# argumentcomputer/multi-stark

Measured on AMD Instinct MI355X. Metric: prove_trace_rows_per_sec, higher is better.
Workload: dtype u64; 1 GPU; U32-add + byte-table lookup (benches/multi_stark.rs), 2^20 additions per proof, bench_config(): log_blowup 2, 100 queries, 10+10 PoW bits, GoldilocksBlake3Config; witness (traces + claims, 64-bit words) in pinned host memory at step start: upload, from_stage_1 on the device and read-back inside the timed region; the library narrows byte-valued traces on host threads INSIDE the step before they cro; rows_per_proof=1048832, proof_bytes=1100053, parallelism=single GPU

## Files before the change

### multi-stark_amd/csrc/host.h

```cpp
#pragma once
#include <memory>
#include <vector>

#include "../../include/mstark.h"
#include "b3_dev.h"
#include "msamd.h"
#include "program.h"

namespace msamd {

void blake3_host(const uint8_t* in, size_t len, uint8_t out[32]);
std::string last_error_text();

struct Challenger {
  std::vector<uint8_t> input, output;
  explicit Challenger(const std::vector<uint8_t>& seed) : input(seed) {}
  void observe_bytes(const uint8_t* p, size_t n) {
    output.clear();
    input.insert(input.end(), p, p + n);
  }
  void observe(u64 v) {
    uint8_t b[8];
    for (int k = 0; k < 8; k++) b[k] = (uint8_t)(v >> (8 * k));
    observe_bytes(b, 8);
// ... 39 lines not shown
  DProgram prog;
  DProgram prefix_prog;
  JitKernel stage2_jit;
  JitKernel stage2_trace_jit;
  bool prefix_on_device = false;
  size_t quotient_degree() const {
    size_t d = (max_constraint_degree > 2 ? max_constraint_degree : 2) - 1, q = 1;
    while (q < d) q <<= 1;
    return q;
  }
};

struct PcsData {
  std::vector<DMat> ldes;
  DTree tree;
};

struct HSystem {
  Ctx* ctx = nullptr;
  Params params;
  std::vector<HCircuit> circuits;
  bool has_pre = false;
  std::vector<Digest> pre_commit;
  std::vector<int> pre_indices;
  PcsData pre_data;
  std::vector<uint8_t> seed;
};
std::unique_ptr<HSystem> system_from_blob(Ctx& ctx, const uint8_t* blob, size_t len);

struct HWitness {
  HSystem* sys = nullptr;
  std::vector<size_t> heights;
  std::vector<DBuf<u64>> traces;
  bool has_remote = false;
  std::vector<DLookups> lookups;
  std::vector<u64> claim_offsets, claim_data;
  size_t claim_elem0 = 0, claim_elems_total = 0;
  std::vector<u64> claim_head;
  bool claims_partial = false;
  DBuf<u64> d_claim_offsets, d_claim_data;
  bool host_resident = false;
  std::vector<const u64*> h_traces;
  std::vector<std::vector<u64>> h_mult, h_args;
  std::vector<void*> registered;
  std::vector<unsigned> pack_bytes;
  std::vector<uint8_t*> h_packed;
  struct Staged {
    bool valid = false, has_host_lookups = false;
    std::vector<DBuf<u64>> traces, mult, args;
    DBuf<u64> claim_offsets, claim_data;
    hipEvent_t ev[3] = {nullptr, nullptr, nullptr};
    void clear() {
      valid = false;
      traces.clear();
      mult.clear();
      args.clear();
      claim_offsets.reset();
      claim_data.reset();
    }
  };
  Staged stage[2];
  int cur = 0;
  bool prefetch = false;
  bool pinned = true;
  void pin(const void* p, size_t bytes);
  HWitness() {}
  HWitness(const HWitness&) = delete;
  HWitness& operator=(const HWitness&) = delete;
  ~HWitness();
};
std::unique_ptr<HWitness> witness_create_host(HSystem& sys, const u64* const* traces, const u64* heights, size_t n_claims,
                                              const u64* claim_offsets, const u64* claim_data, size_t data_first = 0,
                                              size_t data_count = ~size_t(0), const u64* head = nullptr, size_t n_head = 0);
void claims_slice_range(const HSystem& sys, const size_t* heights, size_t n_claims, const u64* offsets, size_t rank, size_t world, size_t& first,
                        size_t& count);
std::unique_ptr<HWitness> witness_create(HSystem& sys, const u64* const* traces, const u64* heights, const u64* const* mult,
                                         const u64* const* args, size_t n_claims, const u64* claim_offsets,
                                         const u64* claim_data);

struct ReadyLookups {
  DBuf<u64> mult, args;
};
std::unique_ptr<HWitness> witness_from_device(HSystem& sys, std::vector<DBuf<u64>>&& traces, const std::vector<size_t>& heights,
                                              DBuf<u64>&& d_claim_offsets, DBuf<u64>&& d_claim_data, size_t n_claims, size_t claim_elems,
                                              std::vector<ReadyLookups>* ready = nullptr);
std::unique_ptr<HWitness> witness_create_device(HSystem& sys, const ms_dev_matrix* traces, size_t n_claims, const u64* claim_offsets,
                                                const u64* claim_data, bool claims_on_device, void* producer_stream);
// ... 50 lines not shown
```

### multi-stark_amd/csrc/msamd.h

```cpp
#pragma once
#include <hip/hip_runtime.h>

#include <algorithm>
#include <cstdint>
#include <cstring>
#include <map>
#include <mutex>
#include <stdexcept>
#include <string>
#include <vector>

#include "gl_dev.h"

namespace msamd {

#define HIP_CHECK(expr)                                                                                   \
  do {                                                                                                    \
    hipError_t _e = (expr);                                                                               \
    if (_e != hipSuccess)                                                                                 \
      throw std::runtime_error(std::string("HIP error: ") + hipGetErrorString(_e) + " at " + __FILE__ + ":" + \
                               std::to_string(__LINE__));                                                 \
  } while (0)

static constexpr unsigned TW_LOG = 28;
// ... 160 lines not shown
  DBuf& operator=(DBuf&& o) noexcept {
    if (this != &o) {
      reset();
      ctx = o.ctx;
      p = o.p;
      n = o.n;
      o.p = nullptr;
    }
    return *this;
  }
  void reset() {
    if (p && ctx) ctx->release(p);
    p = nullptr;
  }
  ~DBuf() { reset(); }
};

struct DMat {
  DBuf<u64> buf;
  size_t h = 0, w = 0;
  u64* d() const { return buf.p; }
};

struct NttSrc {
  const u64* src = nullptr;
  unsigned src_div = 1;
  const u64* scale = nullptr;
};
void ntt_dif(Ctx& ctx, u64* data, unsigned logn, size_t ncols, bool inverse, const NttSrc* from = nullptr, u64 out_mul = 1);
void ntt_dit(Ctx& ctx, u64* data, unsigned logn, size_t ncols, bool inverse, u64 out_mul = 1);
void transpose_in(Ctx& ctx, const u64* rowmajor, u64* colmajor, size_t h, size_t w, bool bitrev_rows);
void transpose_out(Ctx& ctx, const u64* colmajor, u64* rowmajor, size_t h, size_t w, bool bitrev_rows);
void pull_widen_words(const uint8_t* host_packed, unsigned bytes, size_t count, u64* out, hipStream_t stream);
void lde_from_coeffs(Ctx& ctx, const u64* coef, u64* lde, unsigned logn, unsigned log_blowup, size_t w);
void coset_lde(Ctx& ctx, u64* evals_bitrev, u64* lde, unsigned logn, unsigned log_blowup, size_t w);
void quotient_lde(Ctx& ctx, u64* qvals_bitrev, u64* lde, unsigned logn, unsigned logq, unsigned log_blowup, size_t D);

struct MatRef {
  const u64* d;
  uint32_t w;
  uint32_t pad;
  uint64_t stride;
};
struct DTree {
  std::vector<const u64*> mat_d;
  std::vector<size_t> mat_h, mat_w;
  std::vector<size_t> mat_stride;
  DBuf<Digest> digests;
  Digest* ext = nullptr;
  Digest* base() const { return ext ? ext : digests.p; }
  std::vector<size_t> layer_off, layer_len;
  unsigned cap_height = 0;
  size_t max_height() const { return layer_len.empty() ? 0 : layer_len[0]; }
  size_t cap_layer() const {
    size_t L = layer_len.size();
    size_t ch = cap_height < L - 1 ? cap_height : L - 1;
    return L - 1 - ch;
  }
};
void merkle_build(Ctx& ctx, DTree& t);
void merkle_alloc(Ctx& ctx, DTree& t, size_t max_height);
struct FriChallenge;
void merkle_compress_plain(Ctx& ctx, DTree& t, const FriChallenge* fc = nullptr);
std::vector<Digest> merkle_cap(Ctx& ctx, const DTree& t);
void merkle_tree_top(Ctx& ctx, const Digest* d_roots, size_t n, Digest* d_out);
Digest blake3_device(Ctx& ctx, const uint8_t* d_prefix, size_t prefix_len, const u64* d_words, size_t nwords);
// ... 210 lines not shown
```

### multi-stark_amd/csrc/ntt.hip

```cpp
#include <cstring>

#include "msamd.h"

namespace msamd {

namespace {

__device__ __forceinline__ u64 tw_lookup(const u64* __restrict__ t0, const u64* __restrict__ t1, u32 e26) {
  return gl_mul(t1[e26 >> TW_HALF], t0[e26 & ((1u << TW_HALF) - 1)]);
}

template <int DIT>
__device__ __forceinline__ void lds_stages(u64* sm, unsigned k, unsigned logT, const u64* __restrict__ t1) {
  if (k == 0) return;
  const unsigned T = 1u << logT;
  const unsigned nb = (1u << (k - 1)) << logT;
  for (unsigned s = 0; s < k; s++) {
    const unsigned loghalf = DIT ? s : (k - 1 - s);
    const unsigned half = 1u << loghalf;
    const unsigned tsh = TW_HALF - loghalf - 1;
    for (unsigned b = threadIdx.x; b < nb; b += blockDim.x) {
      unsigned l = b & (T - 1), bb = b >> logT;
      unsigned j = bb & (half - 1), grp = bb >> loghalf;
      unsigned i0 = (((grp << (loghalf + 1)) + j) << logT) + l;
// ... 798 lines not shown
    if (sizeof(T) == 1) {
#pragma unroll
      for (int k = 0; k < 4; k++) {
        o[2 * k] = make_ulonglong2(w[k] & 0xff, (w[k] >> 8) & 0xff);
        o[2 * k + 1] = make_ulonglong2((w[k] >> 16) & 0xff, w[k] >> 24);
      }
    } else if (sizeof(T) == 2) {
#pragma unroll
      for (int k = 0; k < 4; k++) o[k] = make_ulonglong2(w[k] & 0xffff, w[k] >> 16);
    } else {
      o[0] = make_ulonglong2(w[0], w[1]);
      o[1] = make_ulonglong2(w[2], w[3]);
    }
  }
  if (blockIdx.x == 0 && threadIdx.x == 0)
    for (size_t k = whole; k < count; k++) out[k] = host[k];
}
}
void pull_widen_words(const uint8_t* host_packed, unsigned bytes, size_t count, u64* out, hipStream_t stream) {
  if (!count) return;
  if (reinterpret_cast<uintptr_t>(host_packed) & 15) throw std::runtime_error("pull_widen_words: source must be 16-byte aligned");
  const dim3 grid((unsigned)std::min<size_t>(256, (count * bytes / 16 + 255) / 256 + 1)), block(256);
  if (bytes == 1)
    hipLaunchKernelGGL(pull_widen_k<uint8_t>, grid, block, 0, stream, host_packed, count, out);
  else if (bytes == 2)
    hipLaunchKernelGGL(pull_widen_k<uint16_t>, grid, block, 0, stream, reinterpret_cast<const uint16_t*>(host_packed), count, out);
  else if (bytes == 4)
    hipLaunchKernelGGL(pull_widen_k<uint32_t>, grid, block, 0, stream, reinterpret_cast<const uint32_t*>(host_packed), count, out);
  else
    throw std::runtime_error("pull_widen_words: unsupported width");
  HIP_CHECK(hipGetLastError());
}

void transpose_out(Ctx& ctx, const u64* colmajor, u64* rowmajor, size_t h, size_t w, bool bitrev_rows) {
  if (h * w == 0) return;
  hipLaunchKernelGGL(transpose_out_k, dim3((unsigned)((h * w + 255) / 256)), dim3(256), 0, ctx.stream, colmajor, rowmajor, h,
                     w, log2_strict(h), bitrev_rows ? 1 : 0);
  HIP_CHECK(hipGetLastError());
}

}
```

### multi-stark_amd/csrc/prover.hip

```cpp
#include <algorithm>
#include <chrono>
#include <cstdio>
#include <cstdlib>

#include <sys/resource.h>
#include <unistd.h>

#include <atomic>
#include <condition_variable>
#include <functional>
#include <mutex>
#include <thread>

#include "host.h"
#include "ingest.h"
#include "lookup_params.h"
#include "open_plan.h"
#include "quotient_params.h"

namespace msamd {

namespace {
void load_block(const uint8_t* p, size_t len, u32 w[16]) {
  uint8_t buf[64];
// ... 127 lines not shown
  size_t n, off = 0;
  u64 word() {
    if (off + 8 > n) throw std::runtime_error("system blob truncated");
    u64 v;
    memcpy(&v, p + off, 8);
    off += 8;
    return v;
  }
};
const u64 BLOB_MAGIC = 0x31305359534D0000ULL;
}

void commit_matrices(Ctx& ctx, std::vector<DMat>&& ldes, unsigned cap_height, PcsData& out) {
  out.ldes = std::move(ldes);
  out.tree = DTree();
  out.tree.cap_height = cap_height;
  for (auto& m : out.ldes) {
    out.tree.mat_d.push_back(m.d());
    out.tree.mat_h.push_back(m.h);
    out.tree.mat_w.push_back(m.w);
  }
  merkle_build(ctx, out.tree);
}

static DMat lde_of_host_matrix(Ctx& ctx, const u64* rowmajor_dev, size_t h, size_t w, unsigned lb) {
  unsigned logn = log2_strict(h);
  DBuf<u64> ev(ctx, h * w);
  transpose_in(ctx, rowmajor_dev, ev.p, h, w, true);
  DMat lde;
  lde.h = h << lb;
  lde.w = w;
  lde.buf = DBuf<u64>(ctx, lde.h * w);
  coset_lde(ctx, ev.p, lde.d(), logn, lb, w);
  return lde;
}

std::unique_ptr<HSystem> system_from_blob(Ctx& ctx, const uint8_t* blob, size_t len) {
  HIP_CHECK(hipSetDevice(ctx.device));
  Reader rd{blob, len};
  if (rd.word() != BLOB_MAGIC) throw std::runtime_error("bad system blob magic");
  std::unique_ptr<HSystem> sys(new HSystem());
  sys->ctx = &ctx;
  Params& p = sys->params;
  p.log_blowup = rd.word();
  p.cap_height = rd.word();
  p.log_final_poly_len = rd.word();
  p.max_log_arity = rd.word();
  p.num_queries = rd.word();
  p.commit_pow_bits = rd.word();
  p.query_pow_bits = rd.word();
  if (p.max_log_arity < 1 || p.max_log_arity > FRI_MAX_LOG_ARITY) throw std::runtime_error("max_log_arity must be 1 .. 6 (a FRI row is hashed as one BLAKE3 chunk)");
  if (p.log_blowup < 1 || p.log_blowup > 8) throw std::runtime_error("log_blowup out of range");
  if (p.commit_pow_bits > 40 || p.query_pow_bits > 40) throw std::runtime_error("proof-of-work bits out of range");
  {
    const char* tag = "multi-stark/v0";
    sys->seed.assign(tag, tag + 14);
    const u64 ps[7] = {p.log_blowup, p.cap_height, p.log_final_poly_len, p.max_log_arity, p.num_queries, p.commit_pow_bits,
                       p.query_pow_bits};
    for (u64 x : ps)
      for (int k = 0; k < 8; k++) sys->seed.push_back((uint8_t)(x >> (8 * k)));
  }
  const size_t D = 2;
  size_t nc = rd.word();
  std::vector<DMat> pre_ldes;
  for (size_t ci = 0; ci < nc; ci++) {
    sys->circuits.emplace_back();
// ... 373 lines not shown
  w->claim_elems_total = tot;
  for (u64 x : w->claim_data)
    if (x >= GL_P) throw std::runtime_error("non-canonical claim value");
  w->d_claim_offsets = DBuf<u64>(ctx, n_claims + 1);
  w->d_claim_data = DBuf<u64>(ctx, std::max<size_t>(tot, 1));
  ctx.h2d(w->d_claim_offsets.p, w->claim_offsets.data(), (n_claims + 1) * 8);
  if (tot) ctx.h2d(w->d_claim_data.p, w->claim_data.data(), tot * 8);
  ctx.sync();
  return w;
}

u64 narrow_range(const u64* in, uint8_t* out, unsigned pb, size_t n);
namespace {
class PackPool {
 public:
  static PackPool* get(int device) {
    static std::mutex mu;
    static std::map<int, PackPool*> pools;
    static const int n_threads = []() {
      int n = 16;
      if (const char* e = getenv("MSAMD_PACK_THREADS")) n = atoi(e);
      return n > 64 ? 64 : n;
    }();
    if (n_threads <= 0) return nullptr;
    std::lock_guard<std::mutex> lk(mu);
    auto it = pools.find(device);
    if (it != pools.end()) return it->second;
    PackPool* p = new PackPool(n_threads);
    pools[device] = p;
    return p;
  }
  static constexpr size_t MAX_CHUNKS = 64, MAX_SUB = 128;
  size_t n_chunks = 0;
  void start(const u64* in, uint8_t* out, unsigned pb, size_t cnt, size_t chunks) {
    job_mu_.lock();
    std::unique_lock<std::mutex> lk(mu_);
    done_cv_.wait(lk, [&] { return busy_ == 0; });
    in_ = in, out_ = out, pb_ = pb, cnt_ = cnt;
    caller_ = std::this_thread::get_id();
    straggle_us_ = getenv("MSAMD_PACK_STRAGGLE_US") ? (unsigned)atoi(getenv("MSAMD_PACK_STRAGGLE_US")) : 0;
    n_chunks = std::max<size_t>(1, std::min(chunks, MAX_CHUNKS));
    per_chunk_ = ((cnt + n_chunks - 1) / n_chunks + 63) & ~size_t(63);
    n_chunks = (cnt + per_chunk_ - 1) / per_chunk_;
    next_.store(0);
    acc_.store(0);
    nsub_ = std::min<size_t>(2 * threads_.size(), MAX_SUB);
    for (size_t k = 0; k < n_chunks; k++) left_[k].store((int)nsub_);
    for (size_t i = 0; i < n_chunks * nsub_; i++) state_[i].store(0, std::memory_order_relaxed);
    busy_ = (int)threads_.size();
    gen_++;
    cv_.notify_all();
  }
  size_t chunk_begin(size_t k) const { return std::min(cnt_, k * per_chunk_); }
  bool wait_chunk(size_t k) {
    double all_claimed_at = 0;
    while (left_[k].load(std::memory_order_acquire) != 0) {
      if (next_.load(std::memory_order_relaxed) >= (k + 1) * nsub_) {
        const double now = now_ms();
        if (all_claimed_at == 0) all_claimed_at = now;
        if (now - all_claimed_at > 0.03) {
          for (size_t sub = 0; sub < nsub_ && left_[k].load(std::memory_order_acquire) != 0; sub++)
            if (state_[k * nsub_ + sub].load(std::memory_order_acquire) != 2) work_piece(k * nsub_ + sub, true);
          continue;
        }
      }
      if (!take_piece()) std::this_thread::yield();
    }
    return (acc_.load() >> (8 * pb_)) == 0;
  }
  void finish() { job_mu_.unlock(); }
  void quiesce() {
    std::unique_lock<std::mutex> lk(mu_);
    done_cv_.wait(lk, [&] { return busy_ == 0; });
  }
  struct Job {
    PackPool& p;
    Job(PackPool& pool, const u64* in, uint8_t* out, unsigned pb, size_t cnt, size_t chunks) : p(pool) { p.start(in, out, pb, cnt, chunks); }
    ~Job() { p.finish(); }
  };

 private:
  explicit PackPool(int n) {
    for (int i = 0; i < n; i++) threads_.emplace_back([this]() { run(); });
    for (auto& t : threads_) t.detach();
  }
  bool take_piece() {
    const size_t it = next_.fetch_add(1);
    if (it >= n_chunks * nsub_) return false;
    work_piece(it, false);
    return true;
  }
  void work_piece(size_t it, bool again) {
    const size_t k = it / nsub_, sub = it % nsub_;
    if (!again) {
      uint8_t unclaimed = 0;
      if (!state_[it].compare_exchange_strong(unclaimed, 1, std::memory_order_acq_rel)) return;
      if (straggle_us_ && sub == 3 && std::this_thread::get_id() != caller_)
        std::this_thread::sleep_for(std::chrono::microseconds(straggle_us_));
    }
    u64 acc = 0;
    const size_t b = chunk_begin(k), e = chunk_begin(k + 1);
    const size_t piece = (((e - b) + nsub_ - 1) / nsub_ + 7) & ~size_t(7);
    const size_t lo = std::min(e, b + sub * piece), hi = std::min(e, lo + piece);
    if (hi > lo) acc = narrow_range(in_ + lo, out_ + lo * pb_, pb_, hi - lo);
    if (acc) acc_.fetch_or(acc);
    if (state_[it].exchange(2, std::memory_order_acq_rel) != 2) left_[k].fetch_sub(1, std::memory_order_release);
  }
  void run() {
    uint64_t seen = 0;
    for (;;) {
      {
        std::unique_lock<std::mutex> lk(mu_);
        cv_.wait(lk, [&] { return gen_ != seen; });
        seen = gen_;
      }
      while (take_piece()) {
      }
      {
        std::unique_lock<std::mutex> lk(mu_);
        if (--busy_ == 0) done_cv_.notify_all();
      }
    }
  }
  std::vector<std::thread> threads_;
  std::mutex mu_, job_mu_;
  std::condition_variable cv_, done_cv_;
  uint64_t gen_ = 0;
  int busy_ = 0;
  const u64* in_ = nullptr;
  uint8_t* out_ = nullptr;
  unsigned pb_ = 1;
  size_t cnt_ = 0, per_chunk_ = 0, nsub_ = 1;
  std::atomic<uint8_t> state_[MAX_CHUNKS * MAX_SUB];
  std::thread::id caller_;
  unsigned straggle_us_ = 0;
  std::atomic<size_t> next_{0};
  std::atomic<u64> acc_{0};
  std::atomic<int> left_[MAX_CHUNKS];
};
}

void HWitness::pin(const void* p, size_t bytes) {
  if (!p || !bytes) return;
  const int r = host_range_pin(p, bytes);
  if (r == 1)
    registered.push_back(const_cast<void*>(p));
  else if (r == 0)
    pinned = false;
}
HWitness::~HWitness() {
  if (!host_resident) return;
  if (sys && sys->ctx) {
    (void)hipSetDevice(sys->ctx->device);
    (void)hipStreamSynchronize(sys->ctx->copy_stream);
    (void)hipStreamSynchronize(sys->ctx->claims_stream);
    if (sys->ctx->side_stream) (void)hipStreamSynchronize(sys->ctx->side_stream);
    (void)hipStreamSynchronize(sys->ctx->main_stream);
  }
  for (auto& st : stage)
    for (auto& e : st.ev)
      if (e) (void)hipEventDestroy(e);
  bool any_packed = false;
  for (uint8_t* p : h_packed) any_packed = any_packed || p != nullptr;
  if (any_packed)
    if (PackPool* pool = PackPool::get(sys && sys->ctx ? sys->ctx->device : 0)) pool->quiesce();
// ... 74 lines not shown
  for (size_t i = 0; i < n_claims; i++)
    if (claim_offsets[i + 1] < claim_offsets[i]) throw std::runtime_error("claim offsets must be non-decreasing");
  const size_t tot = n_claims ? (size_t)claim_offsets[n_claims] : 0;
  w->claim_offsets.assign(claim_offsets, claim_offsets + n_claims + 1);
  w->claim_elems_total = tot;
  if (data_count == ~size_t(0)) {
    w->claim_data.assign(claim_data, claim_data + tot);
  } else {
    if (data_first > tot || data_count > tot - data_first) throw std::runtime_error("claims slice outside the claims' data");
    const size_t need_head = std::min<size_t>(tot, 130);
    if (n_head < need_head || (need_head && !head)) throw std::runtime_error("claims slice: the first 130 elements are needed on every rank");
    w->claims_partial = true;
    w->has_remote = true;
    w->claim_elem0 = data_first;
    w->claim_data.assign(claim_data, claim_data + data_count);
    w->claim_head.assign(head, head + need_head);
    for (u64 x : w->claim_head)
      if (x >= GL_P) throw std::runtime_error("non-canonical claim value");
  }
  for (u64 x : w->claim_data)
    if (x >= GL_P) throw std::runtime_error("non-canonical claim value");
  w->pin(w->claim_offsets.data(), (n_claims + 1) * 8);
  w->pin(w->claim_data.data(), w->claim_data.size() * 8);
  ctx.sync();
  return w;
}

namespace {
struct HostUpload {
  HWitness& w;
  Ctx& ctx;
  bool on = false;
  bool skip_claims = false;
  HostUpload(HWitness& wit, Ctx& c) : w(wit), ctx(c) {}
  bool fused(size_t ci) const {
    const HCircuit& c = w.sys->circuits[ci];
    return w.host_resident && c.stage2_trace_jit.function && w.h_mult[ci].empty();
  }
  void issue(HWitness::Staged& st) {
    HSystem& sys = *w.sys;
    const size_t C = sys.circuits.size();
    for (auto& e : st.ev)
      if (!e) HIP_CHECK(hipEventCreateWithFlags(&e, hipEventDisableTiming));
    st.clear();
    st.traces.resize(C);
    st.mult.resize(C);
    st.args.resize(C);
    HIP_CHECK(hipEventRecord(ctx.copy_ev[3], ctx.stream));
    HIP_CHECK(hipStreamWaitEvent(ctx.copy_stream, ctx.copy_ev[3], 0));
    ctx.side_config();
    ctx.copy_delay();
    HIP_CHECK(hipStreamWaitEvent(ctx.claims_stream, ctx.copy_ev[3], 0));
    const size_t n_claims = w.claim_offsets.size() - 1, tot = w.claim_data.size();
    auto from_caller = [&](void* dst, const void* src, size_t bytes, hipStream_t s) {
      if (w.pinned)
        HIP_CHECK(hipMemcpyAsync(dst, src, bytes, hipMemcpyHostToDevice, s));
      else
        ctx.bounce_h2d(dst, src, bytes, s);
    };
    for (size_t ci = 0; ci < C; ci++) {
      const HCircuit& c = sys.circuits[ci];
      const size_t h = w.heights[ci];
      if (!h || !w.h_traces[ci]) continue;
      const size_t cnt = h * c.main_width;
      st.traces[ci] = DBuf<u64>(ctx, cnt);
      const unsigned pb = w.pack_bytes[ci];
      PackPool* pool = pb && !w.prefetch ? PackPool::get(ctx.device) : nullptr;
      bool sent = false;
      if (pool) {
        static const size_t n_chunks = getenv("MSAMD_PACK_CHUNKS") ? (size_t)atoi(getenv("MSAMD_PACK_CHUNKS")) : 8;
        PackPool::Job job(*pool, w.h_traces[ci], w.h_packed[ci], pb, cnt, n_chunks);
        sent = true;
        for (size_t k = 0; k < pool->n_chunks; k++) {
          if (!pool->wait_chunk(k)) {
            sent = false;
            break;
          }
          if (k == 0) g_probes.mark("narrow upload: first chunk ready");
          const size_t b = pool->chunk_begin(k), e = pool->chunk_begin(k + 1);
          pull_widen_words(w.h_packed[ci] + b * pb, pb, e - b, st.traces[ci].p + b, ctx.copy_stream);
        }
        g_probes.mark("narrow upload: last chunk queued");
      }
      if (!sent) from_caller(st.traces[ci].p, w.h_traces[ci], cnt * 8, ctx.copy_stream);
    }
    HIP_CHECK(hipEventRecord(st.ev[0], ctx.copy_stream));
    st.has_host_lookups = false;
    for (size_t ci = 0; ci < C; ci++) {
      const HCircuit& c = sys.circuits[ci];
      const size_t h = w.heights[ci];
      if (!h || !c.num_lookups || !w.h_traces[ci]) continue;
      if (fused(ci)) continue;
      st.mult[ci] = DBuf<u64>(ctx, h * c.num_lookups);
      st.args[ci] = DBuf<u64>(ctx, std::max<size_t>(h * c.args_width, 1));
      if (!w.h_mult[ci].empty()) {
        st.has_host_lookups = true;
        from_caller(st.mult[ci].p, w.h_mult[ci].data(), w.h_mult[ci].size() * 8, ctx.copy_stream);
        if (!w.h_args[ci].empty()) from_caller(st.args[ci].p, w.h_args[ci].data(), w.h_args[ci].size() * 8, ctx.copy_stream);
      }
    }
    if (!skip_claims) {
      st.claim_offsets = DBuf<u64>(ctx, n_claims + 1);
      st.claim_data = DBuf<u64>(ctx, std::max<size_t>(tot, 1));
      from_caller(st.claim_offsets.p, w.claim_offsets.data(), (n_claims + 1) * 8, ctx.copy_stream);
      if (tot) from_caller(st.claim_data.p, w.claim_data.data(), tot * 8, ctx.copy_stream);
    }
    HIP_CHECK(hipEventRecord(st.ev[2], ctx.copy_stream));
    for (size_t ci = 0; ci < C; ci++) {
      const HCircuit& c = sys.circuits[ci];
      const size_t h = w.heights[ci];
      if (!h || !c.num_lookups || !w.h_mult[ci].empty() || fused(ci) || !w.h_traces[ci]) continue;
      if (!lookup_values_device(ctx, c.prefix_prog, st.traces[ci].p, c.pre_width ? c.d_preprocessed.p : nullptr, h, c.main_width, c.pre_width,
                                c.args_width, st.mult[ci].p, st.args[ci].p, ctx.copy_stream))
        throw std::runtime_error("host-resident witness: lookup prefix does not fit the device sweep");
    }
    HIP_CHECK(hipEventRecord(st.ev[1], ctx.copy_stream));
    st.valid = true;
  }
  void start() {
    if (!w.host_resident) return;
    on = true;
    if (w.prefetch && w.stage[w.cur ^ 1].valid)
      w.cur ^= 1;
    else
      issue(w.stage[w.cur]);
    HWitness::Staged& st = w.stage[w.cur];
    for (size_t ci = 0; ci < st.traces.size(); ci++) {
      w.traces[ci] = std::move(st.traces[ci]);
      w.lookups[ci].mult = std::move(st.mult[ci]);
      w.lookups[ci].args = std::move(st.args[ci]);
    }
    w.d_claim_offsets = std::move(st.claim_offsets);
    w.d_claim_data = std::move(st.claim_data);
    st.valid = false;
    if (w.prefetch) issue(w.stage[w.cur ^ 1]);
  }
  void wait_traces() {
    if (on) HIP_CHECK(hipStreamWaitEvent(ctx.stream, w.stage[w.cur].ev[0], 0));
  }
  void lookup_values() {
    if (!on) return;
    HIP_CHECK(hipStreamWaitEvent(ctx.stream, w.stage[w.cur].ev[1], 0));
    if (ctx.side_forked && ctx.stream != ctx.side_stream) HIP_CHECK(hipStreamWaitEvent(ctx.side_stream, w.stage[w.cur].ev[1], 0));
  }
  void wait_claims() {
    if (on) HIP_CHECK(hipStreamWaitEvent(ctx.stream, w.stage[w.cur].ev[2], 0));
  }
  ~HostUpload() {
    if (!on) return;
    (void)hipStreamSynchronize(ctx.copy_stream);
    (void)hipStreamSynchronize(ctx.claims_stream);
    for (auto& t : w.traces) t.reset();
    for (auto& lk : w.lookups) {
      lk.mult.reset();
      lk.args.reset();
    }
    w.d_claim_offsets.reset();
    w.d_claim_data.reset();
  }
};
}

namespace {
struct PW {
  std::vector<uint8_t> b;
  void u8(uint8_t x) { b.push_back(x); }
  void u64_(u64 x) {
    size_t o = b.size();
    b.resize(o + 8);
    memcpy(&b[o], &x, 8);
  }
  void ext(E2 e) {
    u64_(e.c0);
    u64_(e.c1);
  }
  void raw(const void* p, size_t n) {
    const uint8_t* q = (const uint8_t*)p;
    b.insert(b.end(), q, q + n);
  }
  void cap(const std::vector<Digest>& c) {
    u64_(c.size());
    for (auto& d : c) raw(d.b, 32);
  }
};
typedef std::vector<std::vector<std::vector<E2>>> OpenedRound;
// ... 868 lines not shown
  if (device_claims) {
    s1_cap.assign(ncap, Digest());
    if (sys.has_pre) ch.observe_cap(sys.pre_commit);
    cap_off = ch.input.size();
    ch.observe_cap(s1_cap);
    for (unsigned ld : log_degrees) ch.observe(ld);
    nchunks = blake3_num_chunks(ch.input.size(), claim_words);
    prefix_chunks = std::min(nchunks, (ch.input.size() + 1023) / 1024);
  }
  const bool late_chunk0 = device_claims && prefix_chunks == 1 && nchunks >= 2 && !getenv("MSAMD_OLD_CLAIMS_TREE");
  LateChunk0 late0;
  DBuf<uint8_t> d_prefix;
  auto claims_chunks = [&]() {
    up.wait_claims();
    d_words = DBuf<u64>(ctx, claim_words);
    claims_transcript_words(ctx, wit.d_claim_data.p, wit.d_claim_offsets.p, n_claims, claim_elems, d_words.p);
    d_cvs = DBuf<Digest>(ctx, nchunks);
    blake3_chunk_cvs(ctx, nullptr, ch.input.size(), d_words.p, claim_words, prefix_chunks, nchunks, d_cvs.p);
    d_prefix = DBuf<uint8_t>(ctx, ch.input.size());
    ctx.h2d(d_prefix.p, ch.input.data(), ch.input.size());
    if (late_chunk0) blake3_late_chunk0_prepare(ctx, d_cvs.p, nchunks, late0);
  };

  t0 = now_ms();
  RoctxRange phase("stark/stage1_commit");
  PcsData s1;
  {
    std::vector<DMat> ldes(NA);
    up.wait_traces();
    fork_side();
    for (size_t pos : order) {
      const size_t ci = aidx[pos];
      SideScope sc(ctx, on_side[pos]);
      ldes[pos] = lde_of_host_matrix(ctx, wit.traces[ci].p, wit.heights[ci], sys.circuits[ci].main_width, lb);
    }
    ctx.side_join();
    if (early_claims) {
      ctx.side_fork();
      SideScope sc(ctx, true);
      claims_chunks();
    }
    commit_matrices(ctx, std::move(ldes), (unsigned)prm.cap_height, s1);
  }
  g_probes.mark("stage 1 queued");
  up.wait_claims();
  if (!device_claims) {
    s1_cap = merkle_cap(ctx, s1.tree);
    lap(0);
    if (sys.has_pre) ch.observe_cap(sys.pre_commit);
    ch.observe_cap(s1_cap);
    for (unsigned ld : log_degrees) ch.observe(ld);
    ch.observe((u64)n_claims);
    for (size_t i = 0; i < n_claims; i++) {
      size_t a = wit.claim_offsets[i], b = wit.claim_offsets[i + 1];
      ch.observe((u64)(b - a));
      for (size_t k = a; k < b; k++) ch.observe(wit.claim_data[k]);
    }
  } else {
    lap(0);
    const size_t cl = s1.tree.cap_layer();
    if (s1.tree.layer_len[cl] != ncap) throw std::runtime_error("stage-1 cap size differs from the transcript's placeholder");
    const Digest* d_cap = s1.tree.base() + s1.tree.layer_off[cl];
    if (!early_claims) claims_chunks();
    ctx.side_join();
    od.digest = DBuf<Digest>(ctx, 1);
    if (dev_outer) {
      od.state = DBuf<u32>(ctx, 28);
      d_bg = DBuf<ChallengeBG>(ctx, 1);
    }
// ... 290 lines not shown
```

### multi-stark_amd/csrc/prover_sharded.inc

```

namespace {

struct Comm {
  Ctx& ctx;
  const ms_comm_t* c;
  bool ordered = false;
  const char* phase = "start";
  Comm(Ctx& x, const ms_comm_t* t) : ctx(x), c(t) {
    if (c->set_stream_ordered && !getenv("MSAMD_SHARDED_HOST_SYNC")) {
      if (c->set_stream_ordered(c->user, ctx.main_stream) != 0) throw std::runtime_error("ms_comm.set_stream_ordered failed");
      ordered = true;
    }
  }
  ~Comm() {
    if (ordered) (void)c->set_stream_ordered(c->user, nullptr);
  }
  Comm(const Comm&) = delete;
  Comm& operator=(const Comm&) = delete;
  struct Call {
    Ctx& ctx;
    Call(Comm& cm, const char* what, size_t bytes, size_t detail = 0) : ctx(cm.ctx) {
      char buf[200];
      snprintf(buf, sizeof(buf), "%s: %s (%zu bytes%s%s) on rank %d of %d", cm.phase, what, bytes, detail ? ", part " : "",
               detail ? std::to_string(detail).c_str() : "", cm.rank(), cm.world());
// ... 335 lines not shown
  const size_t total = n_claims ? (size_t)offsets[n_claims] : 0;
  const size_t claim_words = 1 + n_claims + total;
  if (claim_words <= 8192 || world <= 1) {
    first = 0;
    count = total;
    return;
  }
  size_t sl_lo, sl_hi, inv_lo, inv_hi;
  claims_cut(claims_prefix_len(sys, heights), claim_words, n_claims, offsets, world, rank, sl_lo, sl_hi, inv_lo, inv_hi);
  first = (size_t)offsets[sl_lo];
  count = (size_t)offsets[sl_hi] - first;
}

std::vector<uint8_t> prove_sharded(HSystem& sys, HWitness& wit, const ms_comm_t* comm, const int32_t* owners, StageMs* times) {
  Ctx& ctx = *sys.ctx;
  HIP_CHECK(hipSetDevice(ctx.device));
  Comm cm(ctx, comm);
  const Params& prm = sys.params;
  const unsigned lb = (unsigned)prm.log_blowup;
  const size_t C = sys.circuits.size();
  const size_t N = (size_t)cm.world(), me = (size_t)cm.rank();
  const unsigned lw = log2_world(cm.world());
  if (wit.sys != &sys || wit.heights.size() != C) throw std::runtime_error("witness does not belong to this system");
  double t_begin = now_ms(), t0;
  auto lap = [&](int slot) {
    if (times) {
      ctx.sync();
      times->v[slot] = now_ms() - t0;
    }
  };
  PhaseTrace tr(ctx);
  HostUpload up(wit, ctx);
  up.skip_claims = true;
  up.start();
  const size_t n_claims = wit.claim_offsets.size() - 1;
  const size_t claim_elems = wit.claim_elems_total;
  const size_t claim_words = 1 + n_claims + claim_elems;
  DBuf<u64> sl_offs, sl_data;
  size_t sl_lo = 0, sl_hi = 0, inv_lo = 0, inv_hi = 0;
  const bool sliced = wit.host_resident && claim_words > 8192;
  size_t n_active = 0;
  for (size_t i = 0; i < C; i++) n_active += wit.heights[i] > 0;
  size_t max_lde_log = 0;
  for (size_t i = 0; i < C; i++)
    if (wit.heights[i] > 0) max_lde_log = std::max<size_t>(max_lde_log, log2_strict(wit.heights[i]) + lb);
  const size_t cap_digests = size_t(1) << std::min<size_t>((size_t)prm.cap_height, max_lde_log);
  const size_t pl_expected = sys.seed.size() + 8 * (1 + 7 * C) + (sys.has_pre ? 32 * sys.pre_commit.size() : 0) + 32 * cap_digests + 8 * n_active;
  const bool dev_outer = claim_words > 8192 && outer_fits(cap_digests, n_active) && pl_expected <= 1024 &&
                         blake3_num_chunks(pl_expected, claim_words) >= 2 && !getenv("MSAMD_HOST_TRANSCRIPT");
  OuterDev od;
  LateChunk0 late0;
  if (sliced) {
    claims_cut(pl_expected, claim_words, n_claims, wit.claim_offsets.data(), N, me, sl_lo, sl_hi, inv_lo, inv_hi);
    const size_t cnt = sl_hi - sl_lo, o0 = (size_t)wit.claim_offsets[sl_lo], o1 = (size_t)wit.claim_offsets[sl_hi];
    sl_offs = DBuf<u64>(ctx, cnt + 1);
    sl_data = DBuf<u64>(ctx, std::max<size_t>(o1 - o0, 1));
    HIP_CHECK(hipEventRecord(ctx.copy_ev[3], ctx.stream));
    HIP_CHECK(hipStreamWaitEvent(ctx.copy_stream, ctx.copy_ev[3], 0));
    ctx.copy_delay();
    auto from_caller = [&](void* dst, const void* src, size_t bytes) {
      if (wit.pinned)
        HIP_CHECK(hipMemcpyAsync(dst, src, bytes, hipMemcpyHostToDevice, ctx.copy_stream));
      else
        ctx.bounce_h2d(dst, src, bytes, ctx.copy_stream);
    };
    from_caller(sl_offs.p, wit.claim_offsets.data() + sl_lo, (cnt + 1) * 8);
// ... 928 lines not shown
```

Baseline: 161.8 million rows/s.

## Fuse narrow-trace widening with bit-reversed column-major transpose during upload

Adds a kernel that pulls byte-packed trace tiles from pinned host memory and, in one pass, writes both the row-major trace and a bit-reversed column-major copy for the LDE. The host pack pool is changed to narrow rows in a tiled order that matches this kernel, and stage 1 builds the LDE straight from the prepared evaluations, skipping the separate transpose inside lde_of_host_matrix. This overlaps the transpose with the host-to-device transfer, at the cost of an extra full-size device buffer per trace and a more complex, strided access pattern on the host side. The sharded prover keeps the old path.

```diff
diff --git a/multi-stark_amd/csrc/host.h b/multi-stark_amd/csrc/host.h
--- a/multi-stark_amd/csrc/host.h
+++ b/multi-stark_amd/csrc/host.h
@@ -95,6 +95,8 @@
   HSystem* sys = nullptr;
   std::vector<size_t> heights;
   std::vector<DBuf<u64>> traces;
+  std::vector<DBuf<u64>> evals;
+  std::vector<char> evals_ok;
   bool has_remote = false;
   std::vector<DLookups> lookups;
   std::vector<u64> claim_offsets, claim_data;
@@ -111,11 +113,15 @@
   struct Staged {
     bool valid = false, has_host_lookups = false;
     std::vector<DBuf<u64>> traces, mult, args;
+    std::vector<DBuf<u64>> evals;
+    std::vector<char> evals_ok;
     DBuf<u64> claim_offsets, claim_data;
     hipEvent_t ev[3] = {nullptr, nullptr, nullptr};
     void clear() {
       valid = false;
       traces.clear();
+      evals.clear();
+      evals_ok.clear();
       mult.clear();
       args.clear();
       claim_offsets.reset();
diff --git a/multi-stark_amd/csrc/msamd.h b/multi-stark_amd/csrc/msamd.h
--- a/multi-stark_amd/csrc/msamd.h
+++ b/multi-stark_amd/csrc/msamd.h
@@ -216,6 +216,9 @@
 void transpose_in(Ctx& ctx, const u64* rowmajor, u64* colmajor, size_t h, size_t w, bool bitrev_rows);
 void transpose_out(Ctx& ctx, const u64* colmajor, u64* rowmajor, size_t h, size_t w, bool bitrev_rows);
 void pull_widen_words(const uint8_t* host_packed, unsigned bytes, size_t count, u64* out, hipStream_t stream);
+bool pull_widen_transpose_fits(size_t h, size_t w, unsigned bytes);
+void pull_widen_transpose(const uint8_t* host_packed, unsigned bytes, size_t h, size_t w, size_t m_begin, size_t m_end, u64* rowmajor,
+                          u64* colmajor, hipStream_t stream);
 void lde_from_coeffs(Ctx& ctx, const u64* coef, u64* lde, unsigned logn, unsigned log_blowup, size_t w);
 void coset_lde(Ctx& ctx, u64* evals_bitrev, u64* lde, unsigned logn, unsigned log_blowup, size_t w);
 void quotient_lde(Ctx& ctx, u64* qvals_bitrev, u64* lde, unsigned logn, unsigned logq, unsigned log_blowup, size_t D);
diff --git a/multi-stark_amd/csrc/ntt.hip b/multi-stark_amd/csrc/ntt.hip
--- a/multi-stark_amd/csrc/ntt.hip
+++ b/multi-stark_amd/csrc/ntt.hip
@@ -854,6 +854,86 @@
   HIP_CHECK(hipGetLastError());
 }
 
+namespace {
+template <class T>
+__global__ __launch_bounds__(256) void pull_widen_transpose_k(const uint4* __restrict__ host, u64* __restrict__ rowmajor,
+                                                              u64* __restrict__ colmajor, size_t h, u32 w, unsigned logh, u32 m_begin,
+                                                              u32 m_end) {
+  constexpr u32 PER = 16 / sizeof(T), SLAB = 16;
+  __shared__ uint4 stage[16 * SLAB];
+  typedef T __attribute__((may_alias)) TA;
+  const TA* tile = reinterpret_cast<const TA*>(stage);
+  const u32 t = threadIdx.x;
+  const u32 q = w * (u32)sizeof(T);
+  const size_t len = size_t(m_end - m_begin) * q;
+  const size_t items = (len + SLAB - 1) / SLAB;
+  const u32 d16 = 16 / w, s16 = 16 - d16 * w;
+  auto load = [&](size_t item) {
+    const size_t s0 = item * SLAB;
+    const u32 cnt = (u32)min(size_t(SLAB), len - s0);
+    const u32 u = t / cnt, j = t - u * cnt;
+    return t < 16 * cnt ? host[((size_t(u) << (logh - 8)) + m_begin) * q + s0 + j] : make_uint4(0, 0, 0, 0);
+  };
+  size_t item = blockIdx.x;
+  uint4 v = make_uint4(0, 0, 0, 0);
+  if (item < items) v = load(item);
+  for (; item < items; item += gridDim.x) {
+    const size_t s0 = item * SLAB;
+    const u32 cnt = (u32)min(size_t(SLAB), len - s0);
+    if (t < 16 * cnt) stage[t] = v;
+    __syncthreads();
+    if (item + gridDim.x < items) v = load(item + gridDim.x);
+    const u32 ne = cnt * PER;
+    const size_t e0 = s0 * PER;
+    u64* const rm = rowmajor + 16 * size_t(m_begin) * w + e0;
+    if (cnt == SLAB) {
+      constexpr u32 NE = SLAB * PER;
+#pragma unroll
+      for (u32 idx = t; idx < 16 * NE; idx += 256) rm[(size_t(idx / NE) << (logh - 4)) * w + idx % NE] = tile[idx];
+    } else {
+      for (u32 idx = t; idx < 16 * ne; idx += 256) {
+        const u32 u = idx / ne, x = idx - u * ne;
+        rm[(size_t(u) << (logh - 4)) * w + x] = tile[idx];
+      }
+    }
+    {
+      const u32 row0 = (u32)(e0 / w), c0 = (u32)(e0 - size_t(row0) * w);
+      const u32 B = t & 15, u = bitrev32(B, 4);
+      u32 dr = (c0 + (t >> 4)) / w, c = c0 + (t >> 4) - dr * w;
+      for (u32 x = t >> 4; x < ne; x += 16) {
+        const u32 row = row0 + dr, m = m_begin + (row >> 4), a = row & 15;
+        colmajor[size_t(c) * h + ((size_t(bitrev32(a, 4)) << (logh - 4)) | (size_t(bitrev32(m, logh - 8)) << 4) | B)] = tile[u * ne + x];
+        c += s16, dr += d16;
+        if (c >= w) c -= w, dr++;
+      }
+    }
+    __syncthreads();
+  }
+}
+}
+bool pull_widen_transpose_fits(size_t h, size_t w, unsigned bytes) {
+  return h >= 256 && !(h & (h - 1)) && w && w * bytes <= (size_t(1) << 16);
+}
+void pull_widen_transpose(const uint8_t* host_packed, unsigned bytes, size_t h, size_t w, size_t m_begin, size_t m_end, u64* rowmajor,
+                          u64* colmajor, hipStream_t stream) {
+  if (m_begin >= m_end) return;
+  const unsigned logh = log2_strict(h);
+  if (!pull_widen_transpose_fits(h, w, bytes) || m_end > (h >> 8)) throw std::runtime_error("pull_widen_transpose: shape outside the tiled scheme");
+  if (reinterpret_cast<uintptr_t>(host_packed) & 15) throw std::runtime_error("pull_widen_transpose: source must be 16-byte aligned");
+  const size_t items = ((m_end - m_begin) * w * bytes + 15) / 16;
+  const dim3 grid((unsigned)std::min<size_t>(256, items)), block(256);
+  const uint4* src = reinterpret_cast<const uint4*>(host_packed);
+  if (bytes == 1)
+    hipLaunchKernelGGL(pull_widen_transpose_k<uint8_t>, grid, block, 0, stream, src, rowmajor, colmajor, h, (u32)w, logh, (u32)m_begin, (u32)m_end);
+  else if (bytes == 2)
+    hipLaunchKernelGGL(pull_widen_transpose_k<uint16_t>, grid, block, 0, stream, src, rowmajor, colmajor, h, (u32)w, logh, (u32)m_begin, (u32)m_end);
+  else if (bytes == 4)
+    hipLaunchKernelGGL(pull_widen_transpose_k<uint32_t>, grid, block, 0, stream, src, rowmajor, colmajor, h, (u32)w, logh, (u32)m_begin, (u32)m_end);
+  else
+    throw std::runtime_error("pull_widen_transpose: unsupported width");
+  HIP_CHECK(hipGetLastError());
+}
+
 void transpose_out(Ctx& ctx, const u64* colmajor, u64* rowmajor, size_t h, size_t w, bool bitrev_rows) {
   if (h * w == 0) return;
   hipLaunchKernelGGL(transpose_out_k, dim3((unsigned)((h * w + 255) / 256)), dim3(256), 0, ctx.stream, colmajor, rowmajor, h,
diff --git a/multi-stark_amd/csrc/prover.hip b/multi-stark_amd/csrc/prover.hip
--- a/multi-stark_amd/csrc/prover.hip
+++ b/multi-stark_amd/csrc/prover.hip
@@ -183,6 +183,14 @@
   lde.w = w;
   lde.buf = DBuf<u64>(ctx, lde.h * w);
   coset_lde(ctx, ev.p, lde.d(), logn, lb, w);
+  return lde;
+}
+static DMat lde_of_storage_evals(Ctx& ctx, u64* evals_bitrev, size_t h, size_t w, unsigned lb) {
+  DMat lde;
+  lde.h = h << lb;
+  lde.w = w;
+  lde.buf = DBuf<u64>(ctx, lde.h * w);
+  coset_lde(ctx, evals_bitrev, lde.d(), log2_strict(h), lb, w);
   return lde;
 }
 
@@ -622,7 +630,7 @@
   }
   static constexpr size_t MAX_CHUNKS = 64, MAX_SUB = 128;
   size_t n_chunks = 0;
-  void start(const u64* in, uint8_t* out, unsigned pb, size_t cnt, size_t chunks) {
+  void start(const u64* in, uint8_t* out, unsigned pb, size_t cnt, size_t chunks, size_t tile_h = 0) {
     job_mu_.lock();
     std::unique_lock<std::mutex> lk(mu_);
     done_cv_.wait(lk, [&] { return busy_ == 0; });
@@ -630,11 +638,21 @@
     caller_ = std::this_thread::get_id();
     straggle_us_ = getenv("MSAMD_PACK_STRAGGLE_US") ? (unsigned)atoi(getenv("MSAMD_PACK_STRAGGLE_US")) : 0;
     n_chunks = std::max<size_t>(1, std::min(chunks, MAX_CHUNKS));
-    per_chunk_ = ((cnt + n_chunks - 1) / n_chunks + 63) & ~size_t(63);
-    n_chunks = (cnt + per_chunk_ - 1) / per_chunk_;
+    nsub_ = std::min<size_t>(2 * threads_.size(), MAX_SUB);
+    tile_h_ = tile_h;
+    if (tile_h) {
+      const size_t tile_rows = tile_h >> 8;
+      per_chunk_ = (tile_rows + n_chunks - 1) / n_chunks;
+      n_chunks = (tile_rows + per_chunk_ - 1) / per_chunk_;
+      row_words_ = cnt / tile_h;
+      run_parts_ = std::max<size_t>(1, nsub_ / 16);
+      nsub_ = 16 * run_parts_;
+    } else {
+      per_chunk_ = ((cnt + n_chunks - 1) / n_chunks + 63) & ~size_t(63);
+      n_chunks = (cnt + per_chunk_ - 1) / per_chunk_;
+    }
     next_.store(0);
     acc_.store(0);
-    nsub_ = std::min<size_t>(2 * threads_.size(), MAX_SUB);
     for (size_t k = 0; k < n_chunks; k++) left_[k].store((int)nsub_);
     for (size_t i = 0; i < n_chunks * nsub_; i++) state_[i].store(0, std::memory_order_relaxed);
     busy_ = (int)threads_.size();
@@ -642,6 +660,7 @@
     cv_.notify_all();
   }
   size_t chunk_begin(size_t k) const { return std::min(cnt_, k * per_chunk_); }
+  size_t tile_begin(size_t k) const { return std::min(tile_h_ >> 8, k * per_chunk_); }
   bool wait_chunk(size_t k) {
     double all_claimed_at = 0;
     while (left_[k].load(std::memory_order_acquire) != 0) {
@@ -665,7 +684,9 @@
   }
   struct Job {
     PackPool& p;
-    Job(PackPool& pool, const u64* in, uint8_t* out, unsigned pb, size_t cnt, size_t chunks) : p(pool) { p.start(in, out, pb, cnt, chunks); }
+    Job(PackPool& pool, const u64* in, uint8_t* out, unsigned pb, size_t cnt, size_t chunks, size_t tile_h = 0) : p(pool) {
+      p.start(in, out, pb, cnt, chunks, tile_h);
+    }
     ~Job() { p.finish(); }
   };
 
@@ -689,9 +710,17 @@
         std::this_thread::sleep_for(std::chrono::microseconds(straggle_us_));
     }
     u64 acc = 0;
-    const size_t b = chunk_begin(k), e = chunk_begin(k + 1);
-    const size_t piece = (((e - b) + nsub_ - 1) / nsub_ + 7) & ~size_t(7);
-    const size_t lo = std::min(e, b + sub * piece), hi = std::min(e, lo + piece);
+    size_t lo, hi;
+    if (tile_h_) {
+      const size_t rows = 16 * (tile_begin(k + 1) - tile_begin(k)), part_rows = (rows + run_parts_ - 1) / run_parts_;
+      const size_t r0 = std::min(rows, (sub % run_parts_) * part_rows), r1 = std::min(rows, r0 + part_rows);
+      const size_t run_row = (sub / run_parts_) * (tile_h_ >> 4) + 16 * tile_begin(k);
+      lo = (run_row + r0) * row_words_, hi = (run_row + r1) * row_words_;
+    } else {
+      const size_t b = chunk_begin(k), e = chunk_begin(k + 1);
+      const size_t piece = (((e - b) + nsub_ - 1) / nsub_ + 7) & ~size_t(7);
+      lo = std::min(e, b + sub * piece), hi = std::min(e, lo + piece);
+    }
     if (hi > lo) acc = narrow_range(in_ + lo, out_ + lo * pb_, pb_, hi - lo);
     if (acc) acc_.fetch_or(acc);
     if (state_[it].exchange(2, std::memory_order_acq_rel) != 2) left_[k].fetch_sub(1, std::memory_order_release);
@@ -721,6 +750,7 @@
   uint8_t* out_ = nullptr;
   unsigned pb_ = 1;
   size_t cnt_ = 0, per_chunk_ = 0, nsub_ = 1;
+  size_t tile_h_ = 0, row_words_ = 0, run_parts_ = 1;
   std::atomic<uint8_t> state_[MAX_CHUNKS * MAX_SUB];
   std::thread::id caller_;
   unsigned straggle_us_ = 0;
@@ -861,6 +891,7 @@
   Ctx& ctx;
   bool on = false;
   bool skip_claims = false;
+  bool rowmajor_only = false;
   HostUpload(HWitness& wit, Ctx& c) : w(wit), ctx(c) {}
   bool fused(size_t ci) const {
     const HCircuit& c = w.sys->circuits[ci];
@@ -873,6 +904,8 @@
       if (!e) HIP_CHECK(hipEventCreateWithFlags(&e, hipEventDisableTiming));
     st.clear();
     st.traces.resize(C);
+    st.evals.resize(C);
+    st.evals_ok.assign(C, 0);
     st.mult.resize(C);
     st.args.resize(C);
     HIP_CHECK(hipEventRecord(ctx.copy_ev[3], ctx.stream));
@@ -897,8 +930,10 @@
       PackPool* pool = pb && !w.prefetch ? PackPool::get(ctx.device) : nullptr;
       bool sent = false;
       if (pool) {
-        static const size_t n_chunks = getenv("MSAMD_PACK_CHUNKS") ? (size_t)atoi(getenv("MSAMD_PACK_CHUNKS")) : 8;
-        PackPool::Job job(*pool, w.h_traces[ci], w.h_packed[ci], pb, cnt, n_chunks);
+        const size_t n_chunks = getenv("MSAMD_PACK_CHUNKS") ? (size_t)atoi(getenv("MSAMD_PACK_CHUNKS")) : 8;
+        const bool tiled = !rowmajor_only && pull_widen_transpose_fits(h, c.main_width, pb) && !getenv("MSAMD_NO_PULL_TRANSPOSE");
+        if (tiled) st.evals[ci] = DBuf<u64>(ctx, cnt);
+        PackPool::Job job(*pool, w.h_traces[ci], w.h_packed[ci], pb, cnt, n_chunks, tiled ? h : 0);
         sent = true;
         for (size_t k = 0; k < pool->n_chunks; k++) {
           if (!pool->wait_chunk(k)) {
@@ -906,10 +941,16 @@
             break;
           }
           if (k == 0) g_probes.mark("narrow upload: first chunk ready");
-          const size_t b = pool->chunk_begin(k), e = pool->chunk_begin(k + 1);
-          pull_widen_words(w.h_packed[ci] + b * pb, pb, e - b, st.traces[ci].p + b, ctx.copy_stream);
+          if (tiled) {
+            pull_widen_transpose(w.h_packed[ci], pb, h, c.main_width, pool->tile_begin(k), pool->tile_begin(k + 1), st.traces[ci].p,
+                                 st.evals[ci].p, ctx.copy_stream);
+          } else {
+            const size_t b = pool->chunk_begin(k), e = pool->chunk_begin(k + 1);
+            pull_widen_words(w.h_packed[ci] + b * pb, pb, e - b, st.traces[ci].p + b, ctx.copy_stream);
+          }
         }
         g_probes.mark("narrow upload: last chunk queued");
+        st.evals_ok[ci] = sent && tiled;
       }
       if (!sent) from_caller(st.traces[ci].p, w.h_traces[ci], cnt * 8, ctx.copy_stream);
     }
@@ -954,8 +995,11 @@
     else
       issue(w.stage[w.cur]);
     HWitness::Staged& st = w.stage[w.cur];
+    w.evals.resize(st.traces.size());
+    w.evals_ok = st.evals_ok;
     for (size_t ci = 0; ci < st.traces.size(); ci++) {
       w.traces[ci] = std::move(st.traces[ci]);
+      w.evals[ci] = std::move(st.evals[ci]);
       w.lookups[ci].mult = std::move(st.mult[ci]);
       w.lookups[ci].args = std::move(st.args[ci]);
     }
@@ -980,6 +1024,8 @@
     (void)hipStreamSynchronize(ctx.copy_stream);
     (void)hipStreamSynchronize(ctx.claims_stream);
     for (auto& t : w.traces) t.reset();
+    for (auto& t : w.evals) t.reset();
+    w.evals_ok.clear();
     for (auto& lk : w.lookups) {
       lk.mult.reset();
       lk.args.reset();
@@ -1914,9 +1960,15 @@
     for (size_t pos : order) {
       const size_t ci = aidx[pos];
       SideScope sc(ctx, on_side[pos]);
-      ldes[pos] = lde_of_host_matrix(ctx, wit.traces[ci].p, wit.heights[ci], sys.circuits[ci].main_width, lb);
+      if (ci < wit.evals_ok.size() && wit.evals_ok[ci]) {
+        ldes[pos] = lde_of_storage_evals(ctx, wit.evals[ci].p, wit.heights[ci], sys.circuits[ci].main_width, lb);
+        if (!on_side[pos]) wit.evals[ci].reset();
+      } else {
+        ldes[pos] = lde_of_host_matrix(ctx, wit.traces[ci].p, wit.heights[ci], sys.circuits[ci].main_width, lb);
+      }
     }
     ctx.side_join();
+    for (auto& e : wit.evals) e.reset();
     if (early_claims) {
       ctx.side_fork();
       SideScope sc(ctx, true);
diff --git a/multi-stark_amd/csrc/prover_sharded.inc b/multi-stark_amd/csrc/prover_sharded.inc
--- a/multi-stark_amd/csrc/prover_sharded.inc
+++ b/multi-stark_amd/csrc/prover_sharded.inc
@@ -391,6 +391,7 @@
   PhaseTrace tr(ctx);
   HostUpload up(wit, ctx);
   up.skip_claims = true;
+  up.rowmajor_only = true;
   up.start();
   const size_t n_claims = wit.claim_offsets.size() - 1;
   const size_t claim_elems = wit.claim_elems_total;
```

New measurement: 152.4 million rows/s. -5.8%, worse.
